# kykleung/RFS-SLAM

Hardware: AMD Instinct MI355X
Metric: PHD filter-update steps/sec (higher is better)
Workload: dtype f64

## Files before the change

### rfs-slam_amd/csrc/step_fused.h

```cpp
#pragma once
#include "common.h"
#include "update_map.h"
#include "weighting.h"
#include "merge_prune.h"

#include <type_traits>

#ifndef STEP_WPP
#define STEP_WPP 2
#endif
struct StepPredict {
  int mode;
  int nZprev;
  const double *birthPose;
  const double *inPacked;
  int inMask;
};
struct StepLaunchOrder {
  float *cost;
  const int *order;
};
#ifndef STEP_WAVES_PER_EU
#define STEP_WAVES_PER_EU 4
#endif

__host__ __device__ inline size_t step_fused_lds_bytes(int cap, int evalCap, int nZ, int wpp, int gridLog = 5) {
  size_t a = (size_t)RFS_Z_LDS_BYTES + update_map_block_lds_bytes(cap);
  const size_t b = (size_t)RFS_Z_LDS_BYTES + weight_lds_bytes_per_wave(cap, evalCap, nZ) + WEIGHT_SCRATCH_BYTES;
  const size_t c = merge_lds_bytes_per_block(cap, wpp, gridLog);
  if (b > a) a = b;
  if (c > a) a = c;
  return (a + 15) & ~(size_t)15;
}
__host__ __device__ inline size_t step_fused_lds_total(int cap, int evalCap, int nZ, int wpp, int gridLog = 5) {
  return step_fused_lds_bytes(cap, evalCap, nZ, wpp, gridLog) + (((size_t)cap * 2 + 15) & ~(size_t)15);
}

__device__ __forceinline__ void batch_note_capacity(const Buffers &B, const BatchArg &A, const int i, const int bf, const int tid) {
  if (tid != 0) return;
  const int n = __hip_atomic_load(B.count + i, __ATOMIC_RELAXED, __HIP_MEMORY_SCOPE_WORKGROUP);
  if (n < B.cap) return;
  if (__hip_atomic_load(B.err, __ATOMIC_RELAXED, __HIP_MEMORY_SCOPE_AGENT) & ERRBIT_CAPACITY) atomicMin(A.errFilter, bf);
}

template <int WPP, bool PHASE_PRIO, int GL = 5, bool PRED = false, bool BATCH = false>
__global__ __launch_bounds__(WPP * 64) __attribute__((amdgpu_waves_per_eu(STEP_WAVES_PER_EU)))
void phd_step_fused_kernel(Buffers B, Params Parg, int cur, int nZarg, int evalCapArg, int useWeightingArg, MurtyQueue Q,
                           typename std::conditional<BATCH, BatchArg, ZArg>::type zarg, StepPredict SP, StepLaunchOrder SLO) {
  extern __shared__ __align__(16) unsigned char smem_raw[];
  const int tid = threadIdx.x;
  const int lane = tid & 63;
  int i = blockIdx.x;
  unsigned long long tStart = 0ull;
  if constexpr (!PHASE_PRIO) {
    if (SLO.order) i = SLO.order[blockIdx.x];
    if (SLO.cost) tStart = wall_clock64();
  }
  int bf = 0;
  if constexpr (BATCH) bf = __builtin_amdgcn_readfirstlane(i / zarg.nPer);
  const Params &P = [&]() -> const Params & { if constexpr (BATCH) return zarg.params[bf]; else return Parg; }();
  int nZ = nZarg, evalCap = evalCapArg, useWeighting = useWeightingArg;
  if constexpr (BATCH) {
    const BatchFilter &F = zarg.filt[bf];
    nZ = __builtin_amdgcn_readfirstlane(F.nZ);
    evalCap = __builtin_amdgcn_readfirstlane(F.evalCap);
    useWeighting = __builtin_amdgcn_readfirstlane(F.useW);
  }
  if constexpr (PRED) {
    if constexpr (BATCH) {
      Buffers Bp = B;
      Bp.Z = zarg.zPrev + (size_t)bf * (RFSGPU_MAX_Z * 2);
      if (SP.mode) predict_map_particle<WPP * 64>(Bp, P, cur, i, tid, SP.mode > 1, __builtin_amdgcn_readfirstlane(zarg.filt[bf].nZprev), SP.birthPose, true);
    } else {
      if (SP.mode) predict_map_particle<WPP * 64>(B, P, cur, i, tid, SP.mode > 1, SP.nZprev, SP.birthPose, true);
    }
    if (SP.inMask && tid < 13) {
      const double v = SP.inPacked[13 * i + tid];
      if (tid < 3) { if (SP.inMask & 1) B.pose[3 * i + tid] = v; }
      else if (tid < 12) { if (SP.inMask & 2) B.poseCov[9 * i + (tid - 3)] = v; }
      else if (SP.inMask & 4) B.weight[i] = v;
    }
    __threadfence_block();
    __syncthreads();
    __builtin_amdgcn_s_dcache_inv();
    if constexpr (BATCH) batch_note_capacity(B, zarg, i, bf, tid);
  }
  if constexpr (BATCH) {
    if (nZ == 0) {
      const int n = B.count[i];
      for (int pl = 0; pl < PL_COUNT; pl++) {
        const double *src = plane(B.slab[cur], B.cap, i, pl);
        double *dst = plane(B.slab[cur ^ 1], B.cap, i, pl);
        for (int m = tid; m < n; m += WPP * 64) dst[m] = src[m];
      }
      if constexpr (!PHASE_PRIO) {
        if (SLO.cost && threadIdx.x == 0) SLO.cost[i] = 0.f;
      }
      return;
    }
    const double *zs = zarg.z + zarg.filt[bf].zOff;
    stage_measurements_lds(smem_raw, [&](int t) { return zs[t]; }, nZ, tid, WPP * 64);
  } else {
    stage_measurements_lds(smem_raw, [&](int t) { return zarg.v[t]; }, nZ, tid, WPP * 64);
  }
  __syncthreads();
#ifdef RFS_PROFILE
  long long *fd = B.dbg ? B.dbg + 64 + 4 * (size_t)B.N + 4 * (size_t)i : nullptr;
  if (fd && tid == 0) {
    const unsigned hw = __builtin_amdgcn_s_getreg((16 - 1) << 11 | 4), xcc = __builtin_amdgcn_s_getreg((4 - 1) << 11 | 20);
    fd[0] = (long long)((wall_clock64() & 0xfffffffffffull) | ((unsigned long long)(hw & 0xffffu) << 44) | ((unsigned long long)(xcc & 0xfu) << 60));
  }
#endif
  if (WPP == 1) phd_update_map_particle(B, P, cur, nZ, i, lane, smem_raw, smem_raw + RFS_Z_LDS_BYTES);
  else phd_update_map_block<WPP>(B, P, cur, nZ, i, tid, smem_raw, smem_raw + RFS_Z_LDS_BYTES, PHASE_PRIO);
  __threadfence_block();
  __syncthreads();
  if constexpr (BATCH) batch_note_capacity(B, zarg, i, bf, tid);
  RFS_CUT(8);
#ifdef RFS_PROFILE
  if (fd && tid == 0) fd[1] = (long long)wall_clock64();
#endif
  int mergeSrc = cur;
  int tidW = threadIdx.x;
  asm volatile("" : "+v"(tidW));
#ifndef STEP_W_PRIO
#define STEP_W_PRIO 2
#endif
#ifndef STEP_MERGE_PRIO
#define STEP_MERGE_PRIO 1
#endif
  if (PHASE_PRIO) __builtin_amdgcn_s_setprio(STEP_W_PRIO);
  unsigned short *sPerm = reinterpret_cast<unsigned short *>(smem_raw + step_fused_lds_bytes(B.cap, evalCap, nZ, WPP, GL));
  const unsigned short *mergePerm = nullptr;
  if (useWeighting) {
    phd_weight_particle<WPP>(B, P, cur, cur ^ 1, nZ, evalCap, Q, i, tidW, smem_raw, sPerm);
    __threadfence_block();
    __syncthreads();
    mergePerm = sPerm;
  }
  RFS_CUT(16);
  int tidM = threadIdx.x;
  asm volatile("" : "+v"(tidM));
  if (PHASE_PRIO) __builtin_amdgcn_s_setprio(STEP_MERGE_PRIO);
#ifdef RFS_PROFILE
  if (fd && tid == 0) fd[2] = (long long)wall_clock64();
#endif
  gm_merge_particle<WPP, true, GL>(B, P, mergeSrc, mergeSrc ^ 1, i, tidM, smem_raw, mergePerm);
#ifdef RFS_PROFILE
  if (fd && tid == 0) fd[3] = (long long)wall_clock64();
#endif
  if constexpr (!PHASE_PRIO) {
    if (SLO.cost && threadIdx.x == 0) SLO.cost[i] = (float)(wall_clock64() - tStart);
  }
}
```

### rfs-slam_amd/csrc/update_map.h

```cpp
#pragma once
#include "common.h"

struct LmKF {
  double zx0, zx1;
  double i00, i01, i10, i11;
  double factor;
  double k00, k01, k10, k11;
  double p00, p01, p11;
  bool ok;
};

__device__ __forceinline__ void lm_precompute(const Params &P, const PoseReg &pr, double mx, double my, double sxx, double sxy, double syy,
                                              LmKF &k, double &range) {
  MeasOut mo;
  rb_measure(P, pr, mx, my, sxx, sxy, syy, mo);
  range = mo.range;
  k.ok = mo.inRange;
  k.zx0 = mo.z0;
  k.zx1 = mo.z1;
  double det;
  inv2(mo.s00, mo.s01, mo.s10, mo.s11, k.i00, k.i01, k.i10, k.i11, det);
  k.factor = pdf_factor2(det);
  double t00 = sxx * mo.h00 + sxy * mo.h01, t01 = sxx * mo.h10 + sxy * mo.h11;
  double t10 = sxy * mo.h00 + syy * mo.h01, t11 = sxy * mo.h10 + syy * mo.h11;
  k.k00 = t00 * k.i00 + t01 * k.i10;
  k.k01 = t00 * k.i01 + t01 * k.i11;
  k.k10 = t10 * k.i00 + t11 * k.i10;
  k.k11 = t10 * k.i01 + t11 * k.i11;
  double kh00 = k.k00 * mo.h00 + k.k01 * mo.h10, kh01 = k.k00 * mo.h01 + k.k01 * mo.h11;
  double kh10 = k.k10 * mo.h00 + k.k11 * mo.h10, kh11 = k.k10 * mo.h01 + k.k11 * mo.h11;
  double a00 = 1.0 - kh00, a01 = 0.0 - kh01, a10 = 0.0 - kh10, a11 = 1.0 - kh11;
  double q00 = a00 * sxx + a01 * sxy, q01 = a00 * sxy + a01 * syy;
  double q10 = a10 * sxx + a11 * sxy, q11 = a10 * sxy + a11 * syy;
  k.p00 = (q00 + q00) / 2;
  k.p01 = (q01 + q10) / 2;
  k.p11 = (q11 + q11) / 2;
}

__device__ __forceinline__ double pair_weight(const Params &P, const LmKF &k, double pdw, double z0, double z1, double &nu0, double &nu1) {
  if (!k.ok) return 0.0;
  double e0 = z0 - k.zx0, e1 = z1 - k.zx1;
  if (P.kfRange > 0 && fabs(e0) > P.kfRange) return 0.0;
  double w1 = wrap_pi(e1);
  if (P.kfBearing > 0 && fabs(w1) > P.kfBearing) return 0.0;
  nu0 = e0;
  nu1 = w1;
  double t0 = e0 * k.i00 + e1 * k.i10;
  double t1 = e0 * k.i01 + e1 * k.i11;
  double md2 = t0 * e0 + t1 * e1;
  if (md2 > P.newGaussMd2) return 0.0;
  double lik = gauss_from_md2(md2, k.factor);
  if (lik == 0.0) return 0.0;
  return pdw * lik;
}

__host__ __device__ inline size_t update_map_lds_bytes_per_wave(int cap) {
  return (size_t)cap * (8 + 4 + 4) + RFSGPU_MAX_Z * 8;
}

__device__ __forceinline__ bool pair_gate(const Params &P, const LmKF &k, double z0, double z1) {
  const double e0 = z0 - k.zx0;
  if (P.kfRange > 0 && fabs(e0) > P.kfRange) return false;
  const double w1 = wrap_pi(z1 - k.zx1);
  if (P.kfBearing > 0 && fabs(w1) > P.kfBearing) return false;
  return true;
}
__device__ __forceinline__ double pair_md2(const LmKF &k, double z0, double z1) {
  const double e0 = z0 - k.zx0, e1 = z1 - k.zx1;
  const double t0 = e0 * k.i00 + e1 * k.i10;
  const double t1 = e0 * k.i01 + e1 * k.i11;
  return t0 * e0 + t1 * e1;
}
__device__ __forceinline__ double pair_value(const Params &P, const LmKF &k, double pdw, double z0, double z1) {
  const double e0 = z0 - k.zx0, e1 = z1 - k.zx1;
  const double t0 = e0 * k.i00 + e1 * k.i10;
  const double t1 = e0 * k.i01 + e1 * k.i11;
  const double md2 = t0 * e0 + t1 * e1;
  if (md2 > P.newGaussMd2) return 0.0;
  const double lik = gauss_from_md2(md2, k.factor);
  if (lik == 0.0) return 0.0;
  return pdw * lik;
}

typedef float f2_t __attribute__((ext_vector_type(2)));

template <class ZSrc>
__device__ __forceinline__ void stage_measurements_lds(unsigned char *smem_raw, ZSrc zsrc, int nZ, int tid, int nThreads) {
  double *sZ = reinterpret_cast<double *>(smem_raw);
  float *sZf = reinterpret_cast<float *>(smem_raw + 2 * RFSGPU_MAX_Z * 8);
  for (int t = tid; t < 2 * nZ; t += nThreads) sZ[t] = zsrc(t);
  if (tid < 64) {
    float ar = 0.f, ab = 0.f;
    const int z = tid < nZ ? tid : 0;
    const float zr = nZ > 0 ? (float)zsrc(2 * z) : 0.f, zb = nZ > 0 ? (float)zsrc(2 * z + 1) : 0.f;
    sZf[tid] = zr;
    sZf[RFSGPU_MAX_Z + tid] = zb;
    ar = wave_max_f32(fabsf(zr));
    ab = wave_max_f32(fabsf(zb));
    if (tid == 0) { sZf[2 * RFSGPU_MAX_Z] = ar; sZf[2 * RFSGPU_MAX_Z + 1] = ab; }
  }
}

__device__ __forceinline__ unsigned long long gate_candidates(const Params &P, const LmKF &k, const bool live, const int nZ, const float *sZf) {
  const float zx0 = (float)k.zx0, zx1 = (float)k.zx1;
  const float zrMax = sZf[2 * RFSGPU_MAX_Z], zbMax = sZf[2 * RFSGPU_MAX_Z + 1];
  const float inf = __builtin_huge_valf();
  float thrR = (P.kfRange > 0) ? (float)P.kfRange * (1.f + 1e-6f) + 2.5e-7f * (zrMax + fabsf(zx0)) + 1e-30f : inf;
  float thrB = (P.kfBearing > 0) ? (float)P.kfBearing * (1.f + 1e-6f) + 1e-6f * (zbMax + 3.2f) + 1e-6f : inf;
  if (!(zbMax < 50.f)) thrB = inf;
  if (!(zrMax < 1.0e30f)) thrR = inf;
  const f2_t vx0 = {zx0, zx0}, vx1 = {zx1, zx1};
  const f2_t twoPi = {6.2831853071795864769f, 6.2831853071795864769f}, inv2Pi = {0.15915494309189533577f, 0.15915494309189533577f};
  unsigned lo = 0, hi = 0;
#pragma unroll 1
  for (int half = 0; half < 2; half++) {
    const int zBase = 32 * half;
    if (zBase >= nZ) break;
    unsigned bits = 0;
    const f2_t *pr = reinterpret_cast<const f2_t *>(sZf + zBase), *pb = reinterpret_cast<const f2_t *>(sZf + RFSGPU_MAX_Z + zBase);
    const int nPairs = (min(nZ - zBase, 32) + 1) >> 1;
#pragma unroll 4
    for (int q = 0; q < nPairs; q++) {
      const f2_t zr = pr[q], zb = pb[q];
      const f2_t e0 = zr - vx0;
      f2_t w = zb - vx1;
      f2_t kk = w * inv2Pi;
      kk.x = __builtin_rintf(kk.x); kk.y = __builtin_rintf(kk.y);
      w = w - kk * twoPi;
      const bool c0 = ((int)!(fabsf(e0.x) > thrR) & (int)!(fabsf(w.x) > thrB)) != 0;
      const bool c1 = ((int)!(fabsf(e0.y) > thrR) & (int)!(fabsf(w.y) > thrB)) != 0;
      bits |= (c0 ? 1u : 0u) << (2 * q);
      bits |= (c1 ? 2u : 0u) << (2 * q);
    }
    if (half == 0) lo = bits; else hi = bits;
  }
  unsigned long long m = ((unsigned long long)hi << 32) | lo;
  m &= (nZ >= 64) ? ~0ull : ((1ull << nZ) - 1ull);
  return live ? m : 0ull;
}

__device__ __forceinline__ void emit_updated(const LmKF &k, double mx, double my, double z0, double z1, double *pMX, double *pMY, double *pSXX,
                                             double *pSXY, double *pSYY, int pos) {
  const double nu0 = z0 - k.zx0;
  const double nu1 = wrap_pi(z1 - k.zx1);
  pMX[pos] = mx + (k.k00 * nu0 + k.k01 * nu1);
  pMY[pos] = my + (k.k10 * nu0 + k.k11 * nu1);
  pSXX[pos] = k.p00;
  pSXY[pos] = k.p01;
  pSYY[pos] = k.p11;
}

#define UPDMAP_KEEP 4

#ifndef UPDMAP_WAVES_PER_EU
#define UPDMAP_WAVES_PER_EU 2
#endif

__device__ __forceinline__ int compact_appended(const double *sV, int nM, int nSurv, int lane, double *pW, double *pWP, double *pMX, double *pMY,
                                                double *pSXX, double *pSXY, double *pSYY) {
  int out = 0;
  for (int s0 = 0; s0 < nSurv; s0 += 64) {
    const int q = s0 + lane;
    const bool keep = (q < nSurv) && (sV[q] > 0.0);
    const unsigned long long km = __ballot(keep);
    double v0 = 0, v1 = 0, v2 = 0, v3 = 0, v4 = 0, v5 = 0;
    if (keep) { v0 = sV[q]; v1 = pMX[nM + q]; v2 = pMY[nM + q]; v3 = pSXX[nM + q]; v4 = pSXY[nM + q]; v5 = pSYY[nM + q]; }
    __builtin_amdgcn_fence(__ATOMIC_RELEASE, "workgroup");
    wave_sync();
    if (keep) {
      const int d = nM + out + __popcll(km & ((1ull << lane) - 1ull));
      pW[d] = v0; pWP[d] = 0.0; pMX[d] = v1; pMY[d] = v2; pSXX[d] = v3; pSXY[d] = v4; pSYY[d] = v5;
    }
    out += __popcll(km);
  }
  return out;
}

__device__ __forceinline__ void phd_update_map_particle(const Buffers &B, const Params &P, const int cur, const int nZ, const int i,
                                                        const int lane, const unsigned char *smemZ, unsigned char *wb) {
  const double *sZ = reinterpret_cast<const double *>(smemZ);
  const float *sZf = reinterpret_cast<const float *>(smemZ + 2 * RFSGPU_MAX_Z * 8);
  const int cap = B.cap;
  double *sV = reinterpret_cast<double *>(wb);
  double *sCol = sV + cap;
  unsigned *sMZ = reinterpret_cast<unsigned *>(sCol + RFSGPU_MAX_Z);
  unsigned *sSeg = sMZ + cap;

  const int nM = B.count[i];
  const unsigned long long zmask = (nZ >= 64) ? ~0ull : ((1ull << nZ) - 1ull);
  if (nM == 0) {
    if (lane == 0) {
      B.unusedMask[i] = zmask;
      B.nInFov[i] = 0;
    }
    return;
  }
  double *slab = B.slab[cur];
  double *pW = plane(slab, cap, i, PL_W), *pWP = plane(slab, cap, i, PL_WP);
  double *pMX = plane(slab, cap, i, PL_MX), *pMY = plane(slab, cap, i, PL_MY);
  double *pSXX = plane(slab, cap, i, PL_SXX), *pSXY = plane(slab, cap, i, PL_SXY), *pSYY = plane(slab, cap, i, PL_SYY);

  DBG_T(0, 0);
  PoseReg pr;
  load_pose(B, P, i, pr);

  const int nPass = (nM + 63) >> 6;
  const int room = cap - nM;
  int nFov = 0;
  double wsum = 0.0;
  double cs = P.clutter;
  int nSurv = 0;
  bool overflow = false;

  for (int p = 0; p < nPass; p++) {
    const int m = p * 64 + lane;
    const bool act = m < nM;
    double w = 0, mx = 0, my = 0, sxx = 1, sxy = 0, syy = 1;
    if (act) { w = pW[m]; mx = pMX[m]; my = pMY[m]; sxx = pSXX[m]; sxy = pSXY[m]; syy = pSYY[m]; }
    LmKF k;
    double range;
    lm_precompute(P, pr, mx, my, sxx, sxy, syy, k, range);
    bool close;
    double pd = rb_pd(P, range, close);
    if (close) pd = 1;
    const bool fov = act && (pd != 0);
    const double pdw = pd * w;
    nFov += __popcll(__ballot(fov));
    if (P.useCluster) wsum += act ? w : 0.0;
    if (p == 0) DBG_T(0, 4);
    const unsigned long long cand = gate_candidates(P, k, fov && k.ok, nZ, sZf);
    if (p == 0) DBG_T(0, 5);
    unsigned long long surv = 0;
    double keepV[UPDMAP_KEEP];
#pragma unroll
    for (int t = 0; t < UPDMAP_KEEP; t++) keepV[t] = 0.0;
    int cnt = 0;
    unsigned long long gated = 0;
    for (unsigned long long g = cand; g; g &= g - 1) {
      const int z = __builtin_ctzll(g);
      const double z0 = sZ[2 * z], z1 = sZ[2 * z + 1];
      if (!pair_gate(P, k, z0, z1)) continue;
      if (pair_md2(k, z0, z1) > P.newGaussMd2) continue;
      gated |= 1ull << z;
    }
    for (unsigned long long g = gated; g; g &= g - 1) {
      const int z = __builtin_ctzll(g);
      const double z0 = sZ[2 * z], z1 = sZ[2 * z + 1];
      const double v = pair_value(P, k, pdw, z0, z1);
      if (v != 0.0) {
        surv |= (1ull << z);
#pragma unroll
        for (int t = 0; t < UPDMAP_KEEP; t++) keepV[t] = (cnt == t) ? v : keepV[t];
        cnt++;
      }
    }
    if (p == 0) DBG_T(0, 6);
    const int off = wave_excl_scan(cnt, lane);
    const int total = __builtin_amdgcn_readlane(off + cnt, 63);
    if (act) sSeg[m] = ((unsigned)(nSurv + off) << 8) | (unsigned)cnt;
    {
      int pos = nSurv + off, q = 0;
      for (unsigned long long g = surv; g; g &= g - 1, q++, pos++) {
        const int z = __builtin_ctzll(g);
        if (pos < room) {
          const double z0 = sZ[2 * z], z1 = sZ[2 * z + 1];
          double v = keepV[0];
#pragma unroll
          for (int t = 1; t < UPDMAP_KEEP; t++) v = (q == t) ? keepV[t] : v;
          if (q >= UPDMAP_KEEP) v = pair_value(P, k, pdw, z0, z1);
          sV[pos] = v;
          sMZ[pos] = ((unsigned)m << 8) | (unsigned)z;
          emit_updated(k, mx, my, z0, z1, pMX, pMY, pSXX, pSXY, pSYY, nM + pos);
        } else {
          overflow = true;
        }
      }
    }
    wave_sync();
    if (p == 0) DBG_T(0, 7);
    {
      const int lo = nSurv, hi = (nSurv + total < room) ? nSurv + total : room;
      int sIdx = lo;
      for (; sIdx + 4 <= hi; sIdx += 4) {
        const unsigned mz0 = sMZ[sIdx], mz1 = sMZ[sIdx + 1], mz2 = sMZ[sIdx + 2], mz3 = sMZ[sIdx + 3];
        const double v0 = sV[sIdx], v1 = sV[sIdx + 1], v2 = sV[sIdx + 2], v3 = sV[sIdx + 3];
        if ((int)(mz0 & 0xffu) == lane) cs += v0;
        if ((int)(mz1 & 0xffu) == lane) cs += v1;
        if ((int)(mz2 & 0xffu) == lane) cs += v2;
        if ((int)(mz3 & 0xffu) == lane) cs += v3;
      }
      for (; sIdx < hi; sIdx++) {
        const unsigned mz = sMZ[sIdx];
        const double v = sV[sIdx];
        if ((int)(mz & 0xffu) == lane) cs += v;
      }
    }
    nSurv += total;
    if (p == 0) DBG_T(0, 8);
  }
  DBG_T(0, 1);
  if (__ballot(overflow) != 0ull || nSurv > room) {
    if (lane == 0) atomicOr(B.err, ERRBIT_CAPACITY);
    nSurv = room < 0 ? 0 : (nSurv > room ? room : nSurv);
  }
  sCol[lane] = cs;
  wave_sync();

  unsigned long long used = 0;
  bool dropAny = false;
  for (int s0 = 0; s0 < nSurv; s0 += 64) {
    const int sIdx = s0 + lane;
    const bool act = sIdx < nSurv;
    double wn = 0.0;
    int z = 0;
    if (act) { z = (int)(sMZ[sIdx] & 0xffu); wn = sV[sIdx] / sCol[z]; sV[sIdx] = wn; }
    if (act && wn != 0.0) used |= (1ull << z);
    if (act) { pW[nM + sIdx] = wn; pWP[nM + sIdx] = 0.0; }
    dropAny |= act && !(wn > 0.0);
  }
  int outBase = nM + nSurv;
  if (__ballot(dropAny) != 0ull) {
    wave_sync();
    outBase = nM + compact_appended(sV, nM, nSurv, lane, pW, pWP, pMX, pMY, pSXX, pSXY, pSYY);
  }
  wave_sync();

  for (int m = lane; m < nM; m += 64) {
    const double w = pW[m];
    const double dx = pMX[m] - pr.x, dy = pMY[m] - pr.y;
    bool close;
    double pd = rb_pd(P, sqrt(dx * dx + dy * dy), close);
    if (close) pd = 1;
    double w_k = (1 - pd) * w;
    if (close && w > P.birthW) {
      const unsigned seg = sSeg[m];
      const int st = (int)(seg >> 8), c = (int)(seg & 0xffu);
      double rowsum = 0.0;
      for (int q = st; q < st + c && q < nSurv; q++) rowsum += sV[q];
      const double delta_w = pd * w - rowsum;
      if (delta_w > 0) {
        w_k += delta_w;
        if (w_k > 1) w_k = 1;
      }
    }
    pWP[m] = w;
    pW[m] = w_k;
  }
  DBG_T(0, 2);
  used = wave_or_u64(used);
  if (lane == 0) {
    B.count[i] = outBase;
    B.unusedMask[i] = (~used) & zmask;
    B.nInFov[i] = nFov;
  }
  if (P.useCluster) {
    const double s = RFS_DENORM_MIN + wave_sum_dpp(wsum);
    double prod = 1.0;
    for (int z = 0; z < nZ; z++) prod *= readlane_f64(cs, z);
    if (lane == 0) B.weight[i] = exp(s) * prod * B.weight[i];
  }
}

__host__ __device__ inline size_t update_map_block_lds_bytes(int cap) {
  return update_map_lds_bytes_per_wave(cap) + 128;
}

template <int WPP>
__device__ __forceinline__ void phd_update_map_block(const Buffers &B, const Params &P, const int cur, const int nZ, const int i, const int tid,
                                                     const unsigned char *smemZ, unsigned char *wb, const bool phasePrio = false) {
  constexpr int NT = WPP * 64;
  const double *sZ = reinterpret_cast<const double *>(smemZ);
  const float *sZf = reinterpret_cast<const float *>(smemZ + 2 * RFSGPU_MAX_Z * 8);
  const int wave = __builtin_amdgcn_readfirstlane(tid >> 6);
  const int lane = tid & 63;
  const int cap = B.cap;
  double *sV = reinterpret_cast<double *>(wb);
  double *sCol = sV + cap;
  unsigned *sMZ = reinterpret_cast<unsigned *>(sCol + RFSGPU_MAX_Z);
  unsigned *sSeg = sMZ + cap;
  int *sTot = reinterpret_cast<int *>(sSeg + cap);
  int *sMisc = sTot + 16;
  unsigned *sUsed = reinterpret_cast<unsigned *>(sMisc + 4);

  const int nM = B.count[i];
  const unsigned long long zmask = (nZ >= 64) ? ~0ull : ((1ull << nZ) - 1ull);
  if (nM == 0) {
    if (tid == 0) {
      B.unusedMask[i] = zmask;
      B.nInFov[i] = 0;
    }
    return;
  }
  double *slab = B.slab[cur];
  double *pW = plane(slab, cap, i, PL_W), *pWP = plane(slab, cap, i, PL_WP);
  double *pMX = plane(slab, cap, i, PL_MX), *pMY = plane(slab, cap, i, PL_MY);
  double *pSXX = plane(slab, cap, i, PL_SXX), *pSXY = plane(slab, cap, i, PL_SXY), *pSYY = plane(slab, cap, i, PL_SYY);

  PoseReg pr;
  load_pose(B, P, i, pr);
  if (tid < 6) { if (tid < 4) sMisc[tid] = 0; else sUsed[tid - 4] = 0u; }

  const int nPass = (nM + NT - 1) / NT;
  const int room = cap - nM;
  int nFov = 0;
  double cs = P.clutter;
  int nSurv = 0;
  bool overflow = false;

#ifndef STEP_MAP_PRIO
#define STEP_MAP_PRIO 2
#endif
  if (phasePrio) { if ((__builtin_amdgcn_s_getreg((4 - 1) << 11 | 4) & 0xfu) >= 3u) __builtin_amdgcn_s_setprio(3); else __builtin_amdgcn_s_setprio(STEP_MAP_PRIO); }
  for (int p = 0; p < nPass; p++) {
    const int m = p * NT + tid;
    const bool act = m < nM;
    double w = 0, mx = 0, my = 0, sxx = 1, sxy = 0, syy = 1;
    if (act) { w = pW[m]; mx = pMX[m]; my = pMY[m]; sxx = pSXX[m]; sxy = pSXY[m]; syy = pSYY[m]; }
    LmKF k;
    double range;
    lm_precompute(P, pr, mx, my, sxx, sxy, syy, k, range);
    bool close;
    double pd = rb_pd(P, range, close);
    if (close) pd = 1;
    const bool fov = act && (pd != 0);
    const double pdw = pd * w;
    nFov += __popcll(__ballot(fov));
    RFS_CUT(1);
    const unsigned long long cand = gate_candidates(P, k, fov && k.ok, nZ, sZf);
    RFS_CUT(2);
    unsigned long long surv = 0;
    double keepV[UPDMAP_KEEP];
#pragma unroll
    for (int t = 0; t < UPDMAP_KEEP; t++) keepV[t] = 0.0;
    int cnt = 0;
    unsigned long long gated = 0;
    for (unsigned long long g = cand; g; g &= g - 1) {
      const int z = __builtin_ctzll(g);
      const double z0 = sZ[2 * z], z1 = sZ[2 * z + 1];
      if (!pair_gate(P, k, z0, z1)) continue;
      if (pair_md2(k, z0, z1) > P.newGaussMd2) continue;
      gated |= 1ull << z;
    }
    for (unsigned long long g = gated; g; g &= g - 1) {
      const int z = __builtin_ctzll(g);
      const double z0 = sZ[2 * z], z1 = sZ[2 * z + 1];
      const double v = pair_value(P, k, pdw, z0, z1);
      if (v != 0.0) {
        surv |= (1ull << z);
#pragma unroll
        for (int t = 0; t < UPDMAP_KEEP; t++) keepV[t] = (cnt == t) ? v : keepV[t];
        cnt++;
      }
    }
    RFS_CUT(3);
    const int off = wave_excl_scan(cnt, lane);
    const int totalW = __builtin_amdgcn_readlane(off + cnt, 63);
    int *tot = sTot + 8 * (p & 1);
    if (lane == 0) tot[wave] = totalW;
    __syncthreads();
    int before = 0, total = 0;
#pragma unroll
    for (int w2 = 0; w2 < WPP; w2++) { const int t = tot[w2]; before += (w2 < wave) ? t : 0; total += t; }
    if (act) sSeg[m] = ((unsigned)(nSurv + before + off) << 8) | (unsigned)cnt;
    {
      int pos = nSurv + before + off, q = 0;
      for (unsigned long long g = surv; g; g &= g - 1, q++, pos++) {
        const int z = __builtin_ctzll(g);
        if (pos < room) {
          const double z0 = sZ[2 * z], z1 = sZ[2 * z + 1];
          double v = keepV[0];
#pragma unroll
          for (int t = 1; t < UPDMAP_KEEP; t++) v = (q == t) ? keepV[t] : v;
          if (q >= UPDMAP_KEEP) v = pair_value(P, k, pdw, z0, z1);
          sV[pos] = v;
          sMZ[pos] = ((unsigned)m << 8) | (unsigned)z;
          emit_updated(k, mx, my, z0, z1, pMX, pMY, pSXX, pSXY, pSYY, nM + pos);
        } else {
          overflow = true;
        }
      }
    }
    __syncthreads();
    RFS_CUT(4);
    if (wave == 0) {
      const int lo = nSurv, hi = (nSurv + total < room) ? nSurv + total : room;
      int sIdx = lo;
      for (; sIdx + 4 <= hi; sIdx += 4) {
        const unsigned mz0 = sMZ[sIdx], mz1 = sMZ[sIdx + 1], mz2 = sMZ[sIdx + 2], mz3 = sMZ[sIdx + 3];
        const double v0 = sV[sIdx], v1 = sV[sIdx + 1], v2 = sV[sIdx + 2], v3 = sV[sIdx + 3];
        if ((int)(mz0 & 0xffu) == lane) cs += v0;
        if ((int)(mz1 & 0xffu) == lane) cs += v1;
        if ((int)(mz2 & 0xffu) == lane) cs += v2;
        if ((int)(mz3 & 0xffu) == lane) cs += v3;
      }
      for (; sIdx < hi; sIdx++) {
        const unsigned mz = sMZ[sIdx];
        const double v = sV[sIdx];
        if ((int)(mz & 0xffu) == lane) cs += v;
      }
    }
    nSurv += total;
    RFS_CUT(5);
  }
  RFS_CUT(6);
  if (__ballot(overflow) != 0ull && lane == 0) atomicOr(&sMisc[0], 1);
  if (lane == 0) atomicAdd(&sMisc[1], nFov);
  if (wave == 0) sCol[lane] = cs;
  __syncthreads();
  if (sMisc[0] != 0 || nSurv > room) {
    if (tid == 0) atomicOr(B.err, ERRBIT_CAPACITY);
    nSurv = room < 0 ? 0 : (nSurv > room ? room : nSurv);
  }

  {
    unsigned long long used = 0;
    bool dropAny = false;
    for (int s0 = wave * 64; s0 < nSurv; s0 += NT) {
      const int sIdx = s0 + lane;
      const bool act = sIdx < nSurv;
      double wn = 0.0;
      int z = 0;
      if (act) { z = (int)(sMZ[sIdx] & 0xffu); wn = sV[sIdx] / sCol[z]; sV[sIdx] = wn; }
      if (act && wn != 0.0) used |= (1ull << z);
      if (act) { pW[nM + sIdx] = wn; pWP[nM + sIdx] = 0.0; }
      dropAny |= act && !(wn > 0.0);
    }
    used = wave_or_u64(used);
    if (lane == 0) { atomicOr(&sUsed[0], (unsigned)(used & 0xffffffffull)); atomicOr(&sUsed[1], (unsigned)(used >> 32)); }
    if (__ballot(dropAny) != 0ull && lane == 0) atomicOr(&sMisc[2], 1);
  }
  __builtin_amdgcn_fence(__ATOMIC_RELEASE, "workgroup");
  __syncthreads();
  int outBase = nM + nSurv;
  if (sMisc[2] != 0) {
    __builtin_amdgcn_fence(__ATOMIC_ACQUIRE, "workgroup");
    if (wave == 0) {
      const int kept = compact_appended(sV, nM, nSurv, lane, pW, pWP, pMX, pMY, pSXX, pSXY, pSYY);
      if (lane == 0) sMisc[3] = kept;
    }
    __syncthreads();
    outBase = nM + sMisc[3];
  }

  RFS_CUT(7);
  for (int m = tid; m < nM; m += NT) {
    const double w = pW[m];
    const double dx = pMX[m] - pr.x, dy = pMY[m] - pr.y;
    bool close;
    double pd = rb_pd(P, sqrt(dx * dx + dy * dy), close);
    if (close) pd = 1;
    double w_k = (1 - pd) * w;
    if (close && w > P.birthW) {
      const unsigned seg = sSeg[m];
      const int st = (int)(seg >> 8), c = (int)(seg & 0xffu);
      double rowsum = 0.0;
      for (int q = st; q < st + c && q < nSurv; q++) rowsum += sV[q];
      const double delta_w = pd * w - rowsum;
      if (delta_w > 0) {
        w_k += delta_w;
        if (w_k > 1) w_k = 1;
      }
    }
    pWP[m] = w;
    pW[m] = w_k;
  }
  if (tid == 0) {
    B.count[i] = outBase;
    const unsigned long long used = (unsigned long long)sUsed[0] | ((unsigned long long)sUsed[1] << 32);
    B.unusedMask[i] = (~used) & zmask;
    B.nInFov[i] = sMisc[1];
  }
  if (P.useCluster) __syncthreads();
  if (P.useCluster && wave == 0) {
    double wsum = 0.0;
    for (int m = lane; m < nM; m += 64) wsum += pWP[m];
    const double s2 = RFS_DENORM_MIN + wave_sum_dpp(wsum);
    double prod = 1.0;
    for (int z = 0; z < nZ; z++) prod *= readlane_f64(cs, z);
    if (lane == 0) B.weight[i] = exp(s2) * prod * B.weight[i];
  }
}

template <int WPB>
__global__ __launch_bounds__(WPB * 64) __attribute__((amdgpu_waves_per_eu(UPDMAP_WAVES_PER_EU, UPDMAP_WAVES_PER_EU))) void phd_update_map_kernel(Buffers B, Params P, int cur, int nZ, const double *__restrict__ Zg) {
  extern __shared__ __align__(16) unsigned char smem_raw[];
  const int wave = threadIdx.x >> 6;
  const int lane = threadIdx.x & 63;
  stage_measurements_lds(smem_raw, [&](int t) { return Zg[t]; }, nZ, (int)threadIdx.x, WPB * 64);
  __syncthreads();
  const int i = __builtin_amdgcn_readfirstlane(blockIdx.x * WPB + wave);
  if (i >= B.N) return;
  phd_update_map_particle(B, P, cur, nZ, i, lane, smem_raw, smem_raw + RFS_Z_LDS_BYTES + (size_t)wave * update_map_lds_bytes_per_wave(B.cap));
}

template <int WPP>
__global__ __launch_bounds__(WPP * 64) __attribute__((amdgpu_waves_per_eu(UPDMAP_WAVES_PER_EU, 4))) void phd_update_map_block_kernel(Buffers B, Params P, int cur, int nZ, const double *__restrict__ Zg) {
  extern __shared__ __align__(16) unsigned char smem_raw[];
  stage_measurements_lds(smem_raw, [&](int t) { return Zg[t]; }, nZ, (int)threadIdx.x, WPP * 64);
  __syncthreads();
  phd_update_map_block<WPP>(B, P, cur, nZ, (int)blockIdx.x, (int)threadIdx.x, smem_raw, smem_raw + RFS_Z_LDS_BYTES);
}
```

Measured before the change: 9422.

## Redistribute landmark-measurement pair work across wave lanes via LDS pair pool

Replaces the per-lane serial loops over gated measurement candidates with a wave-wide pool. Each (landmark, measurement) pair is written to a per-wave LDS table so all 64 lanes process pairs evenly, fetching the owning lane's Kalman terms by shuffle. Gating, value computation and emission of updated Gaussians all go through this pool. The aim is to remove lane divergence when a few landmarks have many candidates. In exchange it adds LDS per wave, atomics, extra scans and shuffles, and recomputes pair values when more than 64 pairs exist.

```diff
diff --git a/rfs-slam_amd/csrc/step_fused.h b/rfs-slam_amd/csrc/step_fused.h
--- a/rfs-slam_amd/csrc/step_fused.h
+++ b/rfs-slam_amd/csrc/step_fused.h
@@ -25,7 +25,7 @@
 #endif
 
 __host__ __device__ inline size_t step_fused_lds_bytes(int cap, int evalCap, int nZ, int wpp, int gridLog = 5) {
-  size_t a = (size_t)RFS_Z_LDS_BYTES + update_map_block_lds_bytes(cap);
+  size_t a = (size_t)RFS_Z_LDS_BYTES + update_map_block_lds_bytes(cap, wpp);
   const size_t b = (size_t)RFS_Z_LDS_BYTES + weight_lds_bytes_per_wave(cap, evalCap, nZ) + WEIGHT_SCRATCH_BYTES;
   const size_t c = merge_lds_bytes_per_block(cap, wpp, gridLog);
   if (b > a) a = b;
diff --git a/rfs-slam_amd/csrc/update_map.h b/rfs-slam_amd/csrc/update_map.h
--- a/rfs-slam_amd/csrc/update_map.h
+++ b/rfs-slam_amd/csrc/update_map.h
@@ -54,8 +54,15 @@
   return pdw * lik;
 }
 
+#ifndef UPDMAP_POOL_TAB
+#define UPDMAP_POOL_TAB 256
+#endif
+#define UPDMAP_POOL_BYTES (UPDMAP_POOL_TAB * 2 + 64 * 8)
+__host__ __device__ inline size_t update_map_list_bytes(int cap) {
+  return (size_t)cap * (8 + 4 + 4) + RFSGPU_MAX_Z * 8;
+}
 __host__ __device__ inline size_t update_map_lds_bytes_per_wave(int cap) {
-  return (size_t)cap * (8 + 4 + 4) + RFSGPU_MAX_Z * 8;
+  return update_map_list_bytes(cap) + UPDMAP_POOL_BYTES;
 }
 
 __device__ __forceinline__ bool pair_gate(const Params &P, const LmKF &k, double z0, double z1) {
@@ -150,7 +157,152 @@
   pSYY[pos] = k.p11;
 }
 
-#define UPDMAP_KEEP 4
+struct PairPool {
+  unsigned short *tab;
+  unsigned long long *mask;
+};
+__device__ __forceinline__ PairPool pair_pool_at(unsigned char *ws) {
+  PairPool pp;
+  pp.mask = reinterpret_cast<unsigned long long *>(ws);
+  pp.tab = reinterpret_cast<unsigned short *>(ws + 64 * 8);
+  return pp;
+}
+__device__ __forceinline__ void pair_pool_fill(const PairPool &pp, unsigned long long &g, int &pos, const int base, const int lane) {
+  while (g != 0ull && pos < base + UPDMAP_POOL_TAB) {
+    const int z = __builtin_ctzll(g);
+    pp.tab[pos - base] = (unsigned short)(lane | (z << 8));
+    g &= g - 1;
+    pos++;
+  }
+}
+__device__ __forceinline__ double lane_fetch_f64(double v, int srcLane) { return __shfl(v, srcLane, 64); }
+
+__device__ __forceinline__ unsigned long long pool_exact_gates(const Params &P, const LmKF &k, const unsigned long long cand, const double *sZ,
+                                                               const PairPool &pp, const int lane) {
+  const int cnt = __popcll(cand);
+  const int off = wave_excl_scan(cnt, lane);
+  const int total = __builtin_amdgcn_readlane(off + cnt, 63);
+  pp.mask[lane] = 0ull;
+  unsigned long long g = cand;
+  int pos = off;
+  for (int base = 0; base < total; base += UPDMAP_POOL_TAB) {
+    pair_pool_fill(pp, g, pos, base, lane);
+    wave_sync();
+    const int end = min(total - base, UPDMAP_POOL_TAB);
+    for (int t0 = 0; t0 < end; t0 += 64) {
+      const int t = t0 + lane;
+      const bool has = t < end;
+      const unsigned e = has ? (unsigned)pp.tab[t] : (unsigned)lane;
+      const int l = (int)(e & 63u), z = (int)(e >> 8);
+      LmKF kd;
+      kd.zx0 = lane_fetch_f64(k.zx0, l); kd.zx1 = lane_fetch_f64(k.zx1, l);
+      kd.i00 = lane_fetch_f64(k.i00, l); kd.i01 = lane_fetch_f64(k.i01, l);
+      kd.i10 = lane_fetch_f64(k.i10, l); kd.i11 = lane_fetch_f64(k.i11, l);
+      if (has) {
+        const double z0 = sZ[2 * z], z1 = sZ[2 * z + 1];
+        bool pass = pair_gate(P, kd, z0, z1);
+        if (pass && pair_md2(kd, z0, z1) > P.newGaussMd2) pass = false;
+        if (pass) atomicOr(&pp.mask[l], 1ull << z);
+      }
+    }
+    wave_sync();
+  }
+  return pp.mask[lane];
+}
+
+struct PoolKept {
+  unsigned e0;
+  double v0;
+  int total;
+};
+__device__ __forceinline__ double pool_item_value(const Params &P, const LmKF &k, const double pdw, const double *sZ, const bool has, const int l,
+                                                  const int z) {
+  LmKF kd;
+  kd.zx0 = lane_fetch_f64(k.zx0, l); kd.zx1 = lane_fetch_f64(k.zx1, l);
+  kd.i00 = lane_fetch_f64(k.i00, l); kd.i01 = lane_fetch_f64(k.i01, l);
+  kd.i10 = lane_fetch_f64(k.i10, l); kd.i11 = lane_fetch_f64(k.i11, l);
+  kd.factor = lane_fetch_f64(k.factor, l);
+  const double pdwd = lane_fetch_f64(pdw, l);
+  return has ? pair_value(P, kd, pdwd, sZ[2 * z], sZ[2 * z + 1]) : 0.0;
+}
+__device__ __forceinline__ int pool_values(const Params &P, const LmKF &k, const double pdw, const unsigned long long gated, const double *sZ,
+                                           const PairPool &pp, const int lane, PoolKept &kept) {
+  const int cnt = __popcll(gated);
+  const int off = wave_excl_scan(cnt, lane);
+  const int total = __builtin_amdgcn_readlane(off + cnt, 63);
+  kept.e0 = (unsigned)lane;
+  kept.v0 = 0.0;
+  kept.total = total;
+  pp.mask[lane] = 0ull;
+  unsigned long long g = gated;
+  int pos = off;
+  for (int base = 0; base < total; base += UPDMAP_POOL_TAB) {
+    pair_pool_fill(pp, g, pos, base, lane);
+    wave_sync();
+    const int end = min(total - base, UPDMAP_POOL_TAB);
+    for (int t0 = 0; t0 < end; t0 += 64) {
+      const int t = t0 + lane;
+      const bool has = t < end;
+      const unsigned e = has ? (unsigned)pp.tab[t] : (unsigned)lane;
+      const int l = (int)(e & 63u), z = (int)(e >> 8);
+      const double v = pool_item_value(P, k, pdw, sZ, has, l, z);
+      if (v != 0.0) atomicOr(&pp.mask[l], 1ull << z);
+      if (base + t0 == 0) { kept.e0 = e; kept.v0 = v; }
+    }
+    wave_sync();
+  }
+  return __popcll(pp.mask[lane]);
+}
+__device__ __forceinline__ bool pool_emit(const Params &P, const LmKF &k, const double pdw, const double mx, const double my,
+                                          const unsigned long long gated, const double *sZ, const PairPool &pp, const int lane, const PoolKept &kept,
+                                          const int mBase, const int listBase, const int room, const int nM, double *sV, unsigned *sMZ, double *pMX,
+                                          double *pMY, double *pSXX, double *pSXY, double *pSYY) {
+  const int total = kept.total;
+  const bool single = total <= 64;
+  bool overflow = false;
+  int run = listBase;
+  unsigned long long g = gated;
+  int pos = single ? 0 : wave_excl_scan(__popcll(gated), lane);
+  for (int base = 0; base < total; base += UPDMAP_POOL_TAB) {
+    if (!single) {
+      pair_pool_fill(pp, g, pos, base, lane);
+      wave_sync();
+    }
+    const int end = min(total - base, UPDMAP_POOL_TAB);
+    for (int t0 = 0; t0 < end; t0 += 64) {
+      unsigned e = kept.e0;
+      double v = kept.v0;
+      if (!single) {
+        const int t = t0 + lane;
+        const bool has = t < end;
+        e = has ? (unsigned)pp.tab[t] : (unsigned)lane;
+        v = pool_item_value(P, k, pdw, sZ, has, (int)(e & 63u), (int)(e >> 8));
+      }
+      const unsigned long long sm = __ballot(v != 0.0);
+      if (sm == 0ull) continue;
+      const int l = (int)(e & 63u), z = (int)(e >> 8);
+      const int q = run + __popcll(sm & ((1ull << lane) - 1ull));
+      run += __popcll(sm);
+      LmKF kd;
+      kd.zx0 = lane_fetch_f64(k.zx0, l); kd.zx1 = lane_fetch_f64(k.zx1, l);
+      kd.k00 = lane_fetch_f64(k.k00, l); kd.k01 = lane_fetch_f64(k.k01, l);
+      kd.k10 = lane_fetch_f64(k.k10, l); kd.k11 = lane_fetch_f64(k.k11, l);
+      kd.p00 = lane_fetch_f64(k.p00, l); kd.p01 = lane_fetch_f64(k.p01, l); kd.p11 = lane_fetch_f64(k.p11, l);
+      const double mxd = lane_fetch_f64(mx, l), myd = lane_fetch_f64(my, l);
+      if (v != 0.0) {
+        if (q < room) {
+          sV[q] = v;
+          sMZ[q] = ((unsigned)(mBase + l) << 8) | (unsigned)z;
+          emit_updated(kd, mxd, myd, sZ[2 * z], sZ[2 * z + 1], pMX, pMY, pSXX, pSXY, pSYY, nM + q);
+        } else {
+          overflow = true;
+        }
+      }
+    }
+    if (!single) wave_sync();
+  }
+  return overflow;
+}
 
 #ifndef UPDMAP_WAVES_PER_EU
 #define UPDMAP_WAVES_PER_EU 2
@@ -185,6 +337,7 @@
   double *sCol = sV + cap;
   unsigned *sMZ = reinterpret_cast<unsigned *>(sCol + RFSGPU_MAX_Z);
   unsigned *sSeg = sMZ + cap;
+  const PairPool pp = pair_pool_at(wb + update_map_list_bytes(cap));
 
   const int nM = B.count[i];
   const unsigned long long zmask = (nZ >= 64) ? ~0ull : ((1ull << nZ) - 1ull);
@@ -230,52 +383,14 @@
     if (p == 0) DBG_T(0, 4);
     const unsigned long long cand = gate_candidates(P, k, fov && k.ok, nZ, sZf);
     if (p == 0) DBG_T(0, 5);
-    unsigned long long surv = 0;
-    double keepV[UPDMAP_KEEP];
-#pragma unroll
-    for (int t = 0; t < UPDMAP_KEEP; t++) keepV[t] = 0.0;
-    int cnt = 0;
-    unsigned long long gated = 0;
-    for (unsigned long long g = cand; g; g &= g - 1) {
-      const int z = __builtin_ctzll(g);
-      const double z0 = sZ[2 * z], z1 = sZ[2 * z + 1];
-      if (!pair_gate(P, k, z0, z1)) continue;
-      if (pair_md2(k, z0, z1) > P.newGaussMd2) continue;
-      gated |= 1ull << z;
-    }
-    for (unsigned long long g = gated; g; g &= g - 1) {
-      const int z = __builtin_ctzll(g);
-      const double z0 = sZ[2 * z], z1 = sZ[2 * z + 1];
-      const double v = pair_value(P, k, pdw, z0, z1);
-      if (v != 0.0) {
-        surv |= (1ull << z);
-#pragma unroll
-        for (int t = 0; t < UPDMAP_KEEP; t++) keepV[t] = (cnt == t) ? v : keepV[t];
-        cnt++;
-      }
-    }
+    const unsigned long long gated = pool_exact_gates(P, k, cand, sZ, pp, lane);
+    PoolKept kept;
+    const int cnt = pool_values(P, k, pdw, gated, sZ, pp, lane, kept);
     if (p == 0) DBG_T(0, 6);
     const int off = wave_excl_scan(cnt, lane);
     const int total = __builtin_amdgcn_readlane(off + cnt, 63);
     if (act) sSeg[m] = ((unsigned)(nSurv + off) << 8) | (unsigned)cnt;
-    {
-      int pos = nSurv + off, q = 0;
-      for (unsigned long long g = surv; g; g &= g - 1, q++, pos++) {
-        const int z = __builtin_ctzll(g);
-        if (pos < room) {
-          const double z0 = sZ[2 * z], z1 = sZ[2 * z + 1];
-          double v = keepV[0];
-#pragma unroll
-          for (int t = 1; t < UPDMAP_KEEP; t++) v = (q == t) ? keepV[t] : v;
-          if (q >= UPDMAP_KEEP) v = pair_value(P, k, pdw, z0, z1);
-          sV[pos] = v;
-          sMZ[pos] = ((unsigned)m << 8) | (unsigned)z;
-          emit_updated(k, mx, my, z0, z1, pMX, pMY, pSXX, pSXY, pSYY, nM + pos);
-        } else {
-          overflow = true;
-        }
-      }
-    }
+    overflow |= pool_emit(P, k, pdw, mx, my, gated, sZ, pp, lane, kept, p * 64, nSurv, room, nM, sV, sMZ, pMX, pMY, pSXX, pSXY, pSYY);
     wave_sync();
     if (p == 0) DBG_T(0, 7);
     {
@@ -361,8 +476,8 @@
   }
 }
 
-__host__ __device__ inline size_t update_map_block_lds_bytes(int cap) {
-  return update_map_lds_bytes_per_wave(cap) + 128;
+__host__ __device__ inline size_t update_map_block_lds_bytes(int cap, int wpp = 4) {
+  return update_map_list_bytes(cap) + 128 + (size_t)wpp * UPDMAP_POOL_BYTES;
 }
 
 template <int WPP>
@@ -381,6 +496,7 @@
   int *sTot = reinterpret_cast<int *>(sSeg + cap);
   int *sMisc = sTot + 16;
   unsigned *sUsed = reinterpret_cast<unsigned *>(sMisc + 4);
+  const PairPool pp = pair_pool_at(wb + update_map_list_bytes(cap) + 128 + (size_t)wave * UPDMAP_POOL_BYTES);
 
   const int nM = B.count[i];
   const unsigned long long zmask = (nZ >= 64) ? ~0ull : ((1ull << nZ) - 1ull);
@@ -428,30 +544,9 @@
     RFS_CUT(1);
     const unsigned long long cand = gate_candidates(P, k, fov && k.ok, nZ, sZf);
     RFS_CUT(2);
-    unsigned long long surv = 0;
-    double keepV[UPDMAP_KEEP];
-#pragma unroll
-    for (int t = 0; t < UPDMAP_KEEP; t++) keepV[t] = 0.0;
-    int cnt = 0;
-    unsigned long long gated = 0;
-    for (unsigned long long g = cand; g; g &= g - 1) {
-      const int z = __builtin_ctzll(g);
-      const double z0 = sZ[2 * z], z1 = sZ[2 * z + 1];
-      if (!pair_gate(P, k, z0, z1)) continue;
-      if (pair_md2(k, z0, z1) > P.newGaussMd2) continue;
-      gated |= 1ull << z;
-    }
-    for (unsigned long long g = gated; g; g &= g - 1) {
-      const int z = __builtin_ctzll(g);
-      const double z0 = sZ[2 * z], z1 = sZ[2 * z + 1];
-      const double v = pair_value(P, k, pdw, z0, z1);
-      if (v != 0.0) {
-        surv |= (1ull << z);
-#pragma unroll
-        for (int t = 0; t < UPDMAP_KEEP; t++) keepV[t] = (cnt == t) ? v : keepV[t];
-        cnt++;
-      }
-    }
+    const unsigned long long gated = pool_exact_gates(P, k, cand, sZ, pp, lane);
+    PoolKept kept;
+    const int cnt = pool_values(P, k, pdw, gated, sZ, pp, lane, kept);
     RFS_CUT(3);
     const int off = wave_excl_scan(cnt, lane);
     const int totalW = __builtin_amdgcn_readlane(off + cnt, 63);
@@ -462,24 +557,8 @@
 #pragma unroll
     for (int w2 = 0; w2 < WPP; w2++) { const int t = tot[w2]; before += (w2 < wave) ? t : 0; total += t; }
     if (act) sSeg[m] = ((unsigned)(nSurv + before + off) << 8) | (unsigned)cnt;
-    {
-      int pos = nSurv + before + off, q = 0;
-      for (unsigned long long g = surv; g; g &= g - 1, q++, pos++) {
-        const int z = __builtin_ctzll(g);
-        if (pos < room) {
-          const double z0 = sZ[2 * z], z1 = sZ[2 * z + 1];
-          double v = keepV[0];
-#pragma unroll
-          for (int t = 1; t < UPDMAP_KEEP; t++) v = (q == t) ? keepV[t] : v;
-          if (q >= UPDMAP_KEEP) v = pair_value(P, k, pdw, z0, z1);
-          sV[pos] = v;
-          sMZ[pos] = ((unsigned)m << 8) | (unsigned)z;
-          emit_updated(k, mx, my, z0, z1, pMX, pMY, pSXX, pSXY, pSYY, nM + pos);
-        } else {
-          overflow = true;
-        }
-      }
-    }
+    overflow |= pool_emit(P, k, pdw, mx, my, gated, sZ, pp, lane, kept, p * NT + wave * 64, nSurv + before, room, nM, sV, sMZ, pMX, pMY, pSXX, pSXY,
+                          pSYY);
     __syncthreads();
     RFS_CUT(4);
     if (wave == 0) {
```

After: 9537, median of 6. +1.2%, better.
